# Cardinal-Cryptography/zk-apps

Hardware: AMD Instinct MI355X
Metric: shielder_withdraw_groth16_proofs_per_sec_2^20_constraints (higher is better)
Workload: dtype int: signed 28-bit limbs in 32-bit words, 64-bit column accumulators (Fr 255-bit / Fq 381-bit Montgomery); 1 GPU; single withdraw-shaped Groth16 proof, N=2^20 (7 Fr NTTs, 4 G1 MSM + 1 G2 MSM of 2^20-1 terms), 1 proof per step per GPU; relation=update_note (withdraw) with Poseidon-5 hashing, chain-padded to N, curve=BLS12-381, independent_proofs_per_rank=171, distinct_witnesses_per_rank=64, fresh_r_s_per_proof=True, proofs_in_flight_per_gpu=3, msm_schedule=A | B1 (over r*z) + L + H reduced together | B2 (G2)

## Files before the change

include/zkmi_testing.h:

```cpp
#ifndef ZKMI_TESTING_H
#define ZKMI_TESTING_H
#include "zkmi.h"
#ifdef __cplusplus
extern "C" {
#endif

int32_t zkmi_bases_g1_synthetic(zkmi_ctx* ctx, uint64_t n, zkmi_bases_g1** out);
int32_t zkmi_bases_g2_synthetic(zkmi_ctx* ctx, uint64_t n, zkmi_bases_g2** out);
int32_t zkmi_bases_g1_synthetic_range(zkmi_ctx* ctx, uint64_t first, uint64_t n, zkmi_bases_g1** out);
int32_t zkmi_bn254_bases_synthetic(zkmi_ctx* ctx, uint64_t n, zkmi_bn_bases** out);

int32_t zkmi_shielder_r1cs(uint32_t log_n, zkmi_r1cs** out);
int32_t zkmi_shielder_witness(uint32_t log_n, uint64_t seed, uint8_t* out_z );
int32_t zkmi_shielder_witness_from_input(uint32_t log_n, const zkmi_update_note_input* in, uint8_t* out_z);

int32_t zkmi_selftest_fq28(uint64_t seed, uint32_t iters, uint32_t* out_mismatches);
int32_t zkmi_selftest_assembly(uint64_t seed, uint32_t iters, uint32_t* out_mismatches);
int32_t zkmi_selftest_host_pool(uint32_t callers, uint32_t jobs, uint32_t* out_mismatches);
int32_t zkmi_selftest_poseidon(int32_t field, uint64_t seed, uint32_t iters, uint32_t* out_mismatches);
int32_t zkmi_selftest_miller_formulas(const uint8_t g1_affine[96], const uint8_t g2_affine[192], uint8_t out_fq12[576]);
int32_t zkmi_selftest_final_exp_formulas(const uint8_t in_fq12[576], uint8_t out_chain[576], uint8_t out_plain[576]);
int32_t zkmi_verify_each_kernel_ms(float out_ms[3]);
int32_t zkmi_verify_batch_phases(double out_ms[7]);
int32_t zkmi_selftest_quad_add(zkmi_ctx* ctx, uint64_t seed, uint32_t n, uint32_t* out_mismatches);
int32_t zkmi_selftest_msm_g1_sum2_dev(zkmi_ctx* ctx, const void* d_scalars_a, const void* d_scalars_b, uint64_t n,
                                      const zkmi_bases_g1* bases, uint8_t out_affine[96]);

#ifdef __cplusplus
}
#endif
#endif
```

zk-apps_amd/csrc/field28.hpp:

```cpp
#pragma once
#include "field.hpp"

namespace zkmi {

struct Fq28Params {
  static constexpr int NL = 14;
  static constexpr int N32 = 12;
  static constexpr uint32_t INV = 0xffcfffdu;
  static constexpr int32_t MOD[14] = {0xfffaaab, 0xfefffff, 0x3ffffb9, 0xfffeb15, 0x6241eab, 0xa0f6b0f, 0xf6730d2,
                                      0xf38512b, 0x4774b84, 0x4bacd76, 0xba7b643, 0xe69a4b1, 0x1ea397f, 0x001a011};
  static constexpr int32_t ONE[14] = {0x347fcb8, 0xd800000, 0x002b119, 0x0cde6d2, 0xc7212e0, 0x83a2090, 0x037669f,
                                      0xda0f73e, 0x9b09b42, 0x1297bb0, 0x515d98f, 0x012ca7c, 0x659fcfa, 0x000577a};
  static constexpr int32_t R2[14] = {0x10370ed, 0x6d1c345, 0xe243d62, 0xec45c53, 0x3b1d65a, 0x093317d, 0xb4f36a0,
                                     0x5d74088, 0xc10ea72, 0x865d118, 0x7320a75, 0xfd5cd50, 0xcc8a759, 0x000c8d4};
};

struct Fr28Params {
  static constexpr int NL = 10;
  static constexpr int N32 = 8;
  static constexpr uint32_t INV = 0xfffffffu;
  static constexpr int32_t MOD[10] = {0x0000001, 0xffffff0, 0xe5bfeff, 0xa402fff, 0x80553bd,
                                      0x0809a1d, 0x83339d8, 0x299d7d4, 0x3eda753, 0x0000007};
  static constexpr int32_t ONE[10] = {0xdcaaf6c, 0x355093f, 0x8209402, 0x41e37a6, 0x135587d,
                                      0x26172ba, 0x6854f56, 0x3973f39, 0xbc66e55, 0x0000006};
// ... 496 lines not shown
  __device__ __forceinline__ static void mul_cols(int64_t* T, const Fq2P& a, const Fq2P& b, bool negate) {
    constexpr int NL = Fq28::NL;
    const bool o = odd();
    {
      const Fq28 pb = partner(b.v);
      Fq28 X = sel(o, pb, b.v);
      if (negate) X = negl(X);
#pragma unroll
      for (int i = 0; i < NL; i++)
#pragma unroll
        for (int j = 0; j < NL; j++) T[i + j] += (int64_t)a.v.l[i] * X.l[j];
    }
    {
      const Fq28 pa = partner(a.v);
      Fq28 Y = sel(o, b.v, negl(partner(b.v)));
      if (negate) Y = negl(Y);
#pragma unroll
      for (int i = 0; i < NL; i++)
#pragma unroll
        for (int j = 0; j < NL; j++) T[i + j] += (int64_t)pa.l[i] * Y.l[j];
    }
  }
  __device__ __forceinline__ static void operands(const Fq2P& a, const Fq2P& b, bool negate, Fq28& X, Fq28& pa, Fq28& Y) {
    const bool o = odd();
    const Fq28 pb = partner(b.v);
    X = sel(o, pb, b.v);
    Y = sel(o, b.v, negl(pb));
    if (negate) {
      X = negl(X);
      Y = negl(Y);
    }
    pa = partner(a.v);
  }
  __device__ __forceinline__ friend Fq2P operator*(const Fq2P& a, const Fq2P& b) {
#if defined(ZK_FIPS28)
    {
      Fq28 X, pa, Y;
      operands(a, b, false, X, pa, Y);
      return {Fq28::fips<true>(a.v, X, pa, Y)};
    }
#endif
    int64_t T[2 * Fq28::NL];
#pragma unroll
    for (int i = 0; i < 2 * Fq28::NL; i++) T[i] = 0;
    mul_cols(T, a, b, false);
    return {Fq28::reduce(T)};
  }
  __device__ __forceinline__ Fq2P sqr() const {
    const bool o = odd();
    const Fq28 p = partner(v);
    const Fq28 X = sel(o, p.add_lazy(p), v.add_lazy(p));
    const Fq28 Y = sel(o, v, v.sub_lazy(p));
    return {Fq28::mul_inline(X, Y)};
  }
};
__device__ __forceinline__ Fq2P f_mul_sub_mul(const Fq2P& a, const Fq2P& b, const Fq2P& c, const Fq2P& d) {
#if defined(ZK_FIPS28)
  {
    Fq28 X1, pa, Y1, X2, pc, Y2;
    Fq2P::operands(a, b, false, X1, pa, Y1);
    Fq2P::operands(c, d, true, X2, pc, Y2);
    const Fq28* A[4] = {&a.v, &pa, &c.v, &pc};
    const Fq28* B[4] = {&X1, &Y1, &X2, &Y2};
    return {Fq28::fipsn<4>(A, B)};
  }
#endif
  int64_t T[2 * Fq28::NL];
#pragma unroll
  for (int i = 0; i < 2 * Fq28::NL; i++) T[i] = 0;
  Fq2P::mul_cols(T, a, b, false);
  Fq2P::mul_cols(T, c, d, true);
  return {Fq28::reduce(T)};
}
__device__ __forceinline__ Fq2P f_signed_sub_lazy(const Fq2P& a, uint32_t m, const Fq2P& b) {
  Fq28 r;
#pragma unroll
  for (int i = 0; i < Fq28::NL; i++) r.l[i] = (int32_t)(((uint32_t)a.v.l[i] ^ m) - m) - b.v.l[i];
  r.carry();
  return {r};
}
__device__ __forceinline__ Fq2P f_x3(const Fq2P& rr, const Fq2P& ppp, const Fq2P& q) {
  return {f_x3(rr.v, ppp.v, q.v)};
}
#endif

ZK_HD Fq28 fq28_from_fq(const Fq& a) {
  Fq c = a.from_mont();
  return Fq28::from_canonical(c.l);
}
ZK_HD Fq fq_from_fq28(const Fq28& a) {
  Fq c;
  a.to_canonical(c.l);
  return c.to_mont();
}
ZK_HD BnFq28 fq28_from_fq(const BnFq& a) {
  BnFq c = a.from_mont();
  return BnFq28::from_canonical(c.l);
}
ZK_HD BnFq fq_from_fq28(const BnFq28& a) {
  BnFq c;
  a.to_canonical(c.l);
  return c.to_mont();
}
ZK_HD BnFr28 fr28_from_fr(const BnFr& a) {
  BnFr c = a.from_mont();
  return BnFr28::from_canonical(c.l);
}
ZK_HD Fq2_28 fq28_from_fq(const Fq2& a) { return {fq28_from_fq(a.c0), fq28_from_fq(a.c1)}; }
ZK_HD Fq2 fq_from_fq28(const Fq2_28& a) { return {fq_from_fq28(a.c0), fq_from_fq28(a.c1)}; }

}
```

zk-apps_amd/csrc/msm_impl.hpp:

```cpp
#pragma once
#include <stdlib.h>
#include <functional>
#include <type_traits>
#include <vector>
#include "curve.hpp"
#include "host_pool.hpp"
#include "msm.hpp"

namespace zkmi {

static inline uint64_t msm_max_segments(uint64_t buckets) { return (buckets / 16 > (1u << 16) ? buckets / 16 : (1u << 16)) + 1; }
constexpr int MSM_SEG2_LOG = 4;
constexpr uint32_t MSM_SEG2_MIN_SEGS = 256;
constexpr int MSM_TREE_T = 128;
constexpr uint32_t MSM_STAGE_PTS = 16384;
constexpr uint32_t MSM_STAGE_PTS_1 = 4096;
constexpr uint32_t MSM_HEAVY = 256;

template <class T>
__device__ __forceinline__ T load_vec(const T* p) {
  static_assert(sizeof(T) % 16 == 0, "16-byte multiple");
  T r;
  const uint4* s = reinterpret_cast<const uint4*>(p);
  uint4* d = reinterpret_cast<uint4*>(&r);
#pragma unroll
  for (unsigned i = 0; i < sizeof(T) / 16; i++) d[i] = s[i];
  return r;
}
template <class T>
__device__ __forceinline__ void store_vec(T* p, const T& v) {
  static_assert(sizeof(T) % 16 == 0, "16-byte multiple");
  const uint4* s = reinterpret_cast<const uint4*>(&v);
  uint4* d = reinterpret_cast<uint4*>(p);
#pragma unroll
  for (unsigned i = 0; i < sizeof(T) / 16; i++) d[i] = s[i];
}

typedef __attribute__((address_space(3))) void* lds_ptr_t;
typedef const __attribute__((address_space(1))) void* glb_ptr_t;


__device__ __forceinline__ Fq28 ld_comp(const Fq28* p) {
  Fq28 r;
  const uint2* q = reinterpret_cast<const uint2*>(p);
#pragma unroll
  for (int i = 0; i < 7; i++) {
    const uint2 w = q[i];
    r.l[2 * i] = (int32_t)w.x;
    r.l[2 * i + 1] = (int32_t)w.y;
  }
  return r;
}
__device__ __forceinline__ void st_comp(Fq28* p, const Fq28& v) {
  uint2* q = reinterpret_cast<uint2*>(p);
#pragma unroll
  for (int i = 0; i < 7; i++) q[i] = make_uint2((uint32_t)v.l[2 * i], (uint32_t)v.l[2 * i + 1]);
}


template <class F>
__device__ __forceinline__ bool madd_generic(XYZZ<F>& acc, const Affine<F>& p, uint32_t negmask = 0) {
  F pp_ = f_sub_lazy(p.x * acc.zz, acc.x);
  F r = f_signed_sub_lazy(p.y * acc.zzz, negmask, acc.y);
  F pp = pp_.sqr();
  F rr = r.sqr();
  if (pp.is_zero()) return false;
  F ppp = pp_ * pp;
  acc.zz = acc.zz * pp;
  acc.zzz = acc.zzz * ppp;
  F q = acc.x * pp;
  acc.x = f_x3(rr, ppp, q);
  acc.y = f_mul_sub_mul(r, f_sub_lazy(q, acc.x), acc.y, ppp);
  return true;
}
template <class F>
__device__ __forceinline__ bool madd_affine_pair(XYZZ<F>& acc, const Affine<F>& p, uint32_t negmask = 0) {
  F pp_ = f_sub_lazy(p.x, acc.x);
  F r = f_signed_sub_lazy(p.y, negmask, acc.y);
  F pp = pp_.sqr();
  F rr = r.sqr();
  if (pp.is_zero()) return false;
  F ppp = pp_ * pp;
  F q = acc.x * pp;
  acc.x = f_x3(rr, ppp, q);
  acc.y = f_mul_sub_mul(r, f_sub_lazy(q, acc.x), acc.y, ppp);
  acc.zz = pp;
  acc.zzz = ppp;
  return true;
}
template <class P>
__device__ __forceinline__ bool affine_is_zero_words(const Affine<Fp28<P>>& p) {
  if (p.y.l[0] != 0) return false;
  uint32_t o = 0;
#pragma unroll
  for (int i = 0; i < P::NL; i++) o |= (uint32_t)p.x.l[i] | (uint32_t)p.y.l[i];
  return o == 0;
}

constexpr int MSM_MULTI_MAX = 4;
struct SortView {
  const uint32_t *begin, *count, *perm, *sorted;
  uint32_t heavy_thr;
};
template <class F, bool MULTI>
struct AccumArgs;
template <class F>
struct AccumArgs<F, false> {
  const Affine<F>* bases_;
  XYZZ<F>* buckets_;
  uint32_t* redo_;
  SortView sort_;
  __device__ __forceinline__ const Affine<F>* bases() const { return bases_; }
  __device__ __forceinline__ XYZZ<F>* buckets() const { return buckets_; }
  __device__ __forceinline__ uint32_t* redo() const { return redo_; }
  __device__ __forceinline__ const SortView& sort() const { return sort_; }
};
template <class F>
struct AccumArgs<F, true> {
  const Affine<F>* bases_[MSM_MULTI_MAX];
  XYZZ<F>* buckets_[MSM_MULTI_MAX];
  uint32_t* redo_[MSM_MULTI_MAX];
  SortView sort_[MSM_MULTI_MAX];
  __device__ __forceinline__ const Affine<F>* bases() const { return bases_[blockIdx.y]; }
  __device__ __forceinline__ XYZZ<F>* buckets() const { return buckets_[blockIdx.y]; }
  __device__ __forceinline__ uint32_t* redo() const { return redo_[blockIdx.y]; }
  __device__ __forceinline__ const SortView& sort() const { return sort_[blockIdx.y]; }
};
template <class F, int W, int BW, bool MULTI = false, bool INTO = false>
__global__ void __launch_bounds__(64 * BW, W)
k_accum_g1_nc(const AccumArgs<F, MULTI> args, uint32_t total_buckets) {
  const Affine<F>* __restrict__ const bases = args.bases();
  XYZZ<F>* __restrict__ const buckets = args.buckets();
  uint32_t* __restrict__ const redo = args.redo();
  const uint32_t* __restrict__ const begin = args.sort().begin;
  const uint32_t* __restrict__ const count = args.sort().count;
  const uint32_t* __restrict__ const perm = args.sort().perm;
  const uint32_t* __restrict__ const sorted = args.sort().sorted;
  const uint32_t heavy_thr = args.sort().heavy_thr;
  constexpr int CHUNKS = sizeof(Affine<F>) / 16;
  __shared__ uint4 tile[BW][CHUNKS][64];
  const uint32_t t = blockIdx.x * blockDim.x + threadIdx.x;
  const uint32_t wave = threadIdx.x >> 6, lane = threadIdx.x & 63;
  if (t >= total_buckets) return;
  const uint32_t b = perm[t];
  const uint32_t cnt = count[b];
  if (cnt > heavy_thr) return;
  const uint32_t beg = begin[b], end = beg + cnt;
  auto fetch = [&](uint32_t v) {
    const char* src = reinterpret_cast<const char*>(bases + (v & 0x7fffffffu));
#pragma unroll
    for (int q = 0; q < CHUNKS; q++)
      __builtin_amdgcn_global_load_lds((glb_ptr_t)(src + 16 * q), (lds_ptr_t)&tile[wave][q][0], 16, 0, 0);
  };
  auto take = [&](Affine<F>& p) {
    uint4* d = reinterpret_cast<uint4*>(&p);
#pragma unroll
    for (int q = 0; q < CHUNKS; q++) d[q] = tile[wave][q][lane];
    asm volatile("s_waitcnt lgkmcnt(0)" ::: "memory");
  };
  XYZZ<F> acc;
  uint32_t j = beg;
  for (;; j++) {
    if (j >= end) {
      if constexpr (!INTO) store_vec(buckets + b, XYZZ<F>::infinity());
      return;
    }
    const uint32_t v = sorted[j];
    Affine<F> p = load_vec(bases + (v & 0x7fffffffu));
// ... 101 lines not shown
  const uint32_t* __restrict__ const sorted = args.sort().sorted;
  const uint32_t heavy_thr = args.sort().heavy_thr;
  constexpr int CHUNKS = sizeof(Affine<F>) / 16;
  __shared__ uint4 tile[BW][CHUNKS][64];
  const uint32_t gt = blockIdx.x * blockDim.x + threadIdx.x;
  const uint32_t t = gt >> 1, sub = gt & 1u;
  const uint32_t wave = threadIdx.x >> 6, lane = threadIdx.x & 63;
  if (t >= total_buckets) return;
  const uint32_t b = perm[t];
  const uint32_t cnt = count[b];
  if (cnt > heavy_thr) return;
  const uint32_t beg = begin[b], end = beg + cnt;
  auto fetch = [&](uint32_t v) {
    const char* src = reinterpret_cast<const char*>(bases + (v & 0x7fffffffu));
#pragma unroll
    for (int q = 0; q < CHUNKS; q++)
      __builtin_amdgcn_global_load_lds((glb_ptr_t)(src + 16 * q), (lds_ptr_t)&tile[wave][q][0], 16, 0, 0);
  };
  auto take = [&](Affine<F>& p) {
    uint4* d = reinterpret_cast<uint4*>(&p);
#pragma unroll
    for (int q = 0; q < CHUNKS; q++) d[q] = tile[wave][q][lane];
    asm volatile("s_waitcnt lgkmcnt(0)" ::: "memory");
  };
  XYZZ<F> acc = XYZZ<F>::infinity();
  bool has = false, bad = false;
  uint32_t j = beg + sub;
  for (; j < end; j += 2) {
    const uint32_t v = sorted[j];
    Affine<F> p = load_vec(bases + (v & 0x7fffffffu));
    if (affine_is_zero_words(p)) continue;
    if (v >> 31) p.y = p.y.neg();
    acc.x = p.x;
    acc.y = p.y;
    acc.zz = F::one();
    acc.zzz = F::one();
    has = true;
    j += 2;
    break;
  }
  uint32_t v_cur = 0, v_next = 0;
  if (j < end) {
    v_cur = sorted[j];
    fetch(v_cur);
    if (j + 2 < end) v_next = sorted[j + 2];
  }
  for (; j < end; j += 2) {
    Affine<F> p;
    take(p);
    const uint32_t v = v_cur;
    if (j + 2 < end) {
      fetch(v_next);
      v_cur = v_next;
      if (j + 4 < end) v_next = sorted[j + 4];
    }
    if (affine_is_zero_words(p)) continue;
    if (!madd_generic(acc, p, 0u - (v >> 31))) {
      bad = true;
      break;
    }
  }
  const uint32_t flags = (has ? 1u : 0u) | (bad ? 2u : 0u);
  const uint32_t pflags = (uint32_t)__shfl_xor((int)flags, 1);
  XYZZ<F> o;
#pragma unroll
  for (int i = 0; i < F::NL; i++) {
    o.x.l[i] = __shfl_xor(acc.x.l[i], 1);
    o.y.l[i] = __shfl_xor(acc.y.l[i], 1);
    o.zz.l[i] = __shfl_xor(acc.zz.l[i], 1);
    o.zzz.l[i] = __shfl_xor(acc.zzz.l[i], 1);
  }
  if (sub != 0) return;
  bool redo_it = ((flags | pflags) & 2u) != 0;
  if (!redo_it) {
    if (has && (pflags & 1u)) redo_it = !add_generic(acc, o);
    else if (!has) acc = (pflags & 1u) ? o : XYZZ<F>::infinity();
  }
  if (redo_it)
    redo[1 + atomicAdd(redo, 1u)] = b;
  else
    store_vec(buckets + b, acc);
}

template <int W, int BW>
__global__ void __launch_bounds__(64 * BW, W)
k_accum_g2_nc(const Affine<Fq2_28>* __restrict__ bases, const uint32_t* __restrict__ begin,
              const uint32_t* __restrict__ count, const uint32_t* __restrict__ perm,
              const uint32_t* __restrict__ sorted, XYZZ<Fq2_28>* __restrict__ buckets, uint32_t total_buckets,
              uint32_t heavy_thr, uint32_t* __restrict__ redo) {
  const uint32_t gt = blockIdx.x * blockDim.x + threadIdx.x;
  const uint32_t t = gt >> 1, comp = gt & 1u;
  if (t >= total_buckets) return;
  const uint32_t b = perm[t];
  const uint32_t cnt = count[b];
  if (cnt > heavy_thr) return;
  const uint32_t beg = begin[b], end = beg + cnt;
  Fq28* dst = reinterpret_cast<Fq28*>(buckets + b);
  auto load_point = [&](uint32_t v, Affine<Fq2P>& p) {
    const Fq28* src = reinterpret_cast<const Fq28*>(bases + (v & 0x7fffffffu));
    p.x.v = ld_comp(src + comp);
    p.y.v = ld_comp(src + 2 + comp);
    uint32_t o = (uint32_t)p.y.v.l[0];
    o |= (uint32_t)__builtin_amdgcn_mov_dpp((int)o, 0xB1, 0xF, 0xF, true);
    if (o != 0) return false;
#pragma unroll
    for (int i = 0; i < Fq28::NL; i++) o |= (uint32_t)p.x.v.l[i] | (uint32_t)p.y.v.l[i];
    o |= (uint32_t)__builtin_amdgcn_mov_dpp((int)o, 0xB1, 0xF, 0xF, true);
    return o == 0;
  };
  XYZZ<Fq2P> acc;
  uint32_t j = beg;
  for (;; j++) {
    if (j >= end) {
      const Fq28 z = Fq28::zero();
      for (int k = 0; k < 4; k++) st_comp(dst + 2 * k + comp, z);
      return;
    }
    Affine<Fq2P> p;
    const uint32_t v = sorted[j];
    if (load_point(v, p)) continue;
    acc.x = p.x;
    acc.y = (v >> 31) ? p.y.neg() : p.y;
    j++;
    break;
  }
  bool paired = false;
  for (; j < end && !paired; j++) {
    Affine<Fq2P> p;
    const uint32_t v = sorted[j];
    if (load_point(v, p)) continue;
    if (!madd_affine_pair(acc, p, 0u - (v >> 31))) {
      if (comp == 0) redo[1 + atomicAdd(redo, 1u)] = b;
      return;
    }
    paired = true;
  }
  if (!paired) {
    acc.zz = Fq2P::one();
    acc.zzz = Fq2P::one();
  }
  for (; j < end; j++) {
    Affine<Fq2P> p;
    const uint32_t v = sorted[j];
    if (load_point(v, p)) continue;
    if (!madd_generic(acc, p, 0u - (v >> 31))) {
      if (comp == 0) redo[1 + atomicAdd(redo, 1u)] = b;
      return;
    }
  }
  st_comp(dst + comp, acc.x.v);
  st_comp(dst + 2 + comp, acc.y.v);
  st_comp(dst + 4 + comp, acc.zz.v);
  st_comp(dst + 6 + comp, acc.zzz.v);
}

template <int UNUSED = 0>
__global__ void __launch_bounds__(64, 1)
k_accum_g2_split2(const Affine<Fq2_28>* __restrict__ bases, const uint32_t* __restrict__ begin, const uint32_t* __restrict__ count,
                  const uint32_t* __restrict__ perm, const uint32_t* __restrict__ sorted, XYZZ<Fq2_28>* __restrict__ buckets,
                  uint32_t total_buckets, uint32_t heavy_thr, uint32_t* __restrict__ redo) {
  const uint32_t gt = blockIdx.x * blockDim.x + threadIdx.x;
  const uint32_t t = gt >> 2, sub = (gt >> 1) & 1u, comp = gt & 1u;
  if (t >= total_buckets) return;
  const uint32_t b = perm[t];
  const uint32_t cnt = count[b];
  if (cnt > heavy_thr) return;
  const uint32_t beg = begin[b], end = beg + cnt;
  Fq28* dst = reinterpret_cast<Fq28*>(buckets + b);
  auto load_point = [&](uint32_t v, Affine<Fq2P>& p) {
    const Fq28* src = reinterpret_cast<const Fq28*>(bases + (v & 0x7fffffffu));
    p.x.v = ld_comp(src + comp);
    p.y.v = ld_comp(src + 2 + comp);
    uint32_t o = (uint32_t)p.y.v.l[0];
    o |= (uint32_t)__builtin_amdgcn_mov_dpp((int)o, 0xB1, 0xF, 0xF, true);
    if (o != 0) return false;
#pragma unroll
    for (int i = 0; i < Fq28::NL; i++) o |= (uint32_t)p.x.v.l[i] | (uint32_t)p.y.v.l[i];
    o |= (uint32_t)__builtin_amdgcn_mov_dpp((int)o, 0xB1, 0xF, 0xF, true);
    return o == 0;
  };
  XYZZ<Fq2P> acc = XYZZ<Fq2P>::infinity();
  bool has = false, bad = false;
  uint32_t j = beg + sub;
  for (; j < end; j += 2) {
    Affine<Fq2P> p;
    const uint32_t v = sorted[j];
    if (load_point(v, p)) continue;
    acc.x = p.x;
    acc.y = (v >> 31) ? p.y.neg() : p.y;
    acc.zz = Fq2P::one();
    acc.zzz = Fq2P::one();
    has = true;
    j += 2;
    break;
  }
  for (; j < end; j += 2) {
    Affine<Fq2P> p;
    const uint32_t v = sorted[j];
    if (load_point(v, p)) continue;
    if (!madd_generic(acc, p, 0u - (v >> 31))) {
      bad = true;
      break;
    }
  }
  const uint32_t flags = (has ? 1u : 0u) | (bad ? 2u : 0u);
  const uint32_t pflags = (uint32_t)__shfl_xor((int)flags, 2);
  XYZZ<Fq2P> o;
#pragma unroll
  for (int i = 0; i < Fq28::NL; i++) {
    o.x.v.l[i] = __shfl_xor(acc.x.v.l[i], 2);
    o.y.v.l[i] = __shfl_xor(acc.y.v.l[i], 2);
    o.zz.v.l[i] = __shfl_xor(acc.zz.v.l[i], 2);
    o.zzz.v.l[i] = __shfl_xor(acc.zzz.v.l[i], 2);
  }
  if (sub != 0) return;
  bool redo_it = ((flags | pflags) & 2u) != 0;
  if (!redo_it) {
    if (has && (pflags & 1u)) redo_it = !add_generic(acc, o);
    else if (!has) acc = (pflags & 1u) ? o : XYZZ<Fq2P>::infinity();
  }
  if (redo_it) {
    if (comp == 0) redo[1 + atomicAdd(redo, 1u)] = b;
  } else {
    st_comp(dst + comp, acc.x.v);
    st_comp(dst + 2 + comp, acc.y.v);
    st_comp(dst + 4 + comp, acc.zz.v);
    st_comp(dst + 6 + comp, acc.zzz.v);
  }
}

template <class F>
// ... 229 lines not shown
    for (int q = 0; q < CHUNKS; q++) __builtin_amdgcn_global_load_lds((glb_ptr_t)(src + 16 * q), (lds_ptr_t)&tile[q][0], 16, 0, 0);
  };
  auto take = [&](Affine<F>& p) {
    uint4* d = reinterpret_cast<uint4*>(&p);
#pragma unroll
    for (int q = 0; q < CHUNKS; q++) d[q] = tile[q][lane];
    asm volatile("s_waitcnt lgkmcnt(0)" ::: "memory");
  };
  for (uint32_t it = blockIdx.x; it < n_items; it += gridDim.x) {
    const uint32_t e = heavy_plan_entry(ent, n_ent, it);
    const uint32_t beg = ent[4 * e + 1], cnt = ent[4 * e + 2], first = ent[4 * e + 3];
    const uint32_t w0 = beg + (it - first) * 64u * pl;
    const uint32_t w1 = (w0 + 64u * pl < beg + cnt) ? w0 + 64u * pl : beg + cnt;
    XYZZ<F>* const dst = pool + (size_t)it * 64 + lane;
    XYZZ<F> acc;
    uint32_t j = w0 + lane;
    bool have = false;
    for (; j < w1; j += 64) {
      const uint32_t v = sorted[j];
      Affine<F> p = load_vec(bases + (v & 0x7fffffffu));
      if (affine_is_zero_words(p)) continue;
      if (v >> 31) p.y = p.y.neg();
      acc.x = p.x;
      acc.y = p.y;
      have = true;
      j += 64;
      break;
    }
    if (!have) {
      store_vec(dst, XYZZ<F>::infinity());
      continue;
    }
    uint32_t v_cur = 0, v_next = 0;
    if (j < w1) {
      v_cur = sorted[j];
      fetch(v_cur);
      if (j + 64 < w1) v_next = sorted[j + 64];
    }
    bool bad = false, paired = false;
    if (j < w1) {
      Affine<F> p;
      take(p);
      const uint32_t v = v_cur;
      if (j + 64 < w1) {
        fetch(v_next);
        v_cur = v_next;
        if (j + 128 < w1) v_next = sorted[j + 128];
      }
      j += 64;
      if (!affine_is_zero_words(p)) {
        bad = !madd_affine_pair(acc, p, 0u - (v >> 31));
        paired = true;
      }
    }
    if (!paired) {
      acc.zz = F::one();
      acc.zzz = F::one();
    }
    if (bad) j = w1;
    for (; j < w1; j += 64) {
      Affine<F> p;
      take(p);
      const uint32_t v = v_cur;
      if (j + 64 < w1) {
        fetch(v_next);
        v_cur = v_next;
        if (j + 128 < w1) v_next = sorted[j + 128];
      }
      if (affine_is_zero_words(p)) continue;
      if (!madd_generic(acc, p, 0u - (v >> 31))) {
        bad = true;
        break;
      }
    }
    if (bad) store_vec(dst, heavy_marker<F>());
    else store_vec(dst, acc);
  }
}

template <int W>
__global__ void __launch_bounds__(64, W)
k_accum_heavy_nc_g2(const Affine<Fq2_28>* __restrict__ bases, const uint32_t* __restrict__ sorted, const uint32_t* __restrict__ hplan,
                    XYZZ<Fq2_28>* __restrict__ pool) {
  if (hplan[3] != 0) return;
  const uint32_t n_items = hplan[0], pl = hplan[1], n_ent = hplan[2];
  const uint32_t* __restrict__ const ent = hplan + 4;
  const uint32_t pair = threadIdx.x >> 1, comp = threadIdx.x & 1u;
  auto load_point = [&](uint32_t v, Affine<Fq2P>& p) {
    const Fq28* src = reinterpret_cast<const Fq28*>(bases + (v & 0x7fffffffu));
    p.x.v = ld_comp(src + comp);
    p.y.v = ld_comp(src + 2 + comp);
    uint32_t o = (uint32_t)p.y.v.l[0];
    o |= (uint32_t)__builtin_amdgcn_mov_dpp((int)o, 0xB1, 0xF, 0xF, true);
    if (o != 0) return false;
#pragma unroll
    for (int i = 0; i < Fq28::NL; i++) o |= (uint32_t)p.x.v.l[i] | (uint32_t)p.y.v.l[i];
    o |= (uint32_t)__builtin_amdgcn_mov_dpp((int)o, 0xB1, 0xF, 0xF, true);
    return o == 0;
  };
  for (uint32_t it = blockIdx.x; it < n_items; it += gridDim.x) {
    const uint32_t e = heavy_plan_entry(ent, n_ent, it);
    const uint32_t beg = ent[4 * e + 1], cnt = ent[4 * e + 2], first = ent[4 * e + 3];
    const uint32_t w0 = beg + (it - first) * 32u * pl;
    const uint32_t w1 = (w0 + 32u * pl < beg + cnt) ? w0 + 32u * pl : beg + cnt;
    Fq28* const dst = reinterpret_cast<Fq28*>(pool + (size_t)it * 32 + pair);
    XYZZ<Fq2P> acc;
    uint32_t j = w0 + pair;
    bool have = false, bad = false;
    for (; j < w1; j += 32) {
      Affine<Fq2P> p;
      const uint32_t v = sorted[j];
      if (load_point(v, p)) continue;
      acc.x = p.x;
      acc.y = (v >> 31) ? p.y.neg() : p.y;
      have = true;
      j += 32;
      break;
    }
    if (have) {
      bool paired = false;
      for (; j < w1 && !paired && !bad; j += 32) {
        Affine<Fq2P> p;
        const uint32_t v = sorted[j];
        if (load_point(v, p)) continue;
        if (madd_affine_pair(acc, p, 0u - (v >> 31))) paired = true;
        else bad = true;
      }
      if (!paired) {
        acc.zz = Fq2P::one();
        acc.zzz = Fq2P::one();
      }
      for (; j < w1 && !bad; j += 32) {
        Affine<Fq2P> p;
        const uint32_t v = sorted[j];
        if (load_point(v, p)) continue;
        if (!madd_generic(acc, p, 0u - (v >> 31))) bad = true;
      }
    }
    if (!have || bad) {
      const Fq28 z = Fq28::zero();
      Fq28 mk = z;
      mk.l[0] = (bad && comp == 0) ? 1 : 0;
      st_comp(dst + comp, z);
      st_comp(dst + 2 + comp, z);
      st_comp(dst + 4 + comp, z);
      st_comp(dst + 6 + comp, mk);
    } else {
      st_comp(dst + comp, acc.x.v);
      st_comp(dst + 2 + comp, acc.y.v);
      st_comp(dst + 4 + comp, acc.zz.v);
      st_comp(dst + 6 + comp, acc.zzz.v);
    }
  }
}

constexpr uint32_t MSM_HSPLIT_MAX = 1024;
constexpr uint32_t MSM_HPOOL = MSM_HEAVY_CAP * MSM_HSPLIT;
__device__ __forceinline__ uint32_t heavy_nsplit(uint32_t h, uint32_t count, uint32_t pts, uint32_t item0) {
  if (h >= MSM_HEAVY_CAP) return 1u;
  uint32_t n = (count + pts - 1) / pts;
  n = n < 1 ? 1 : (n > MSM_HSPLIT_MAX ? MSM_HSPLIT_MAX : n);
  if (item0 + n > MSM_HPOOL) n = 1;
  return n;
}
template <class L>
__device__ __forceinline__ void accum_heavy_body(const typename L::Base* __restrict__ bases, const uint32_t* __restrict__ begin,
                                                 const uint32_t* __restrict__ count, const uint32_t* __restrict__ heavy,
                                                 const uint32_t* __restrict__ sorted, typename L::Stored* __restrict__ buckets,
                                                 typename L::Stored* __restrict__ heavy_partial, uint32_t* __restrict__ ticket,
                                                 uint32_t into, uint32_t h_first, uint32_t h_limit, const uint32_t* __restrict__ hplan,
                                                 const typename L::Stored* __restrict__ pool_nc) {
  typedef typename L::P P;
  extern __shared__ __align__(16) unsigned char lds_raw[];
  typename L::Stored* sh = reinterpret_cast<typename L::Stored*>(lds_raw);
  __shared__ uint32_t is_last;
  const uint32_t pt = threadIdx.x / L::LANES, comp = threadIdx.x % L::LANES, npt = blockDim.x / L::LANES;
  constexpr uint32_t PER_ITEM = 64 / L::LANES;
  const bool pmode = hplan != nullptr && hplan[3] == 0;
  const uint32_t* __restrict__ const ent = hplan + 4;
  const uint32_t pl_nc = pmode ? hplan[1] : 0u;
  auto partial_at = [&](uint32_t h, uint32_t j) {
    P v = L::load(pool_nc + j, comp);
    bool empty;
    if (L::is_marker(v, comp, &empty)) {
      const uint32_t it = j / PER_ITEM, ln = j % PER_ITEM;
      const uint32_t beg = ent[4 * h + 1], cnt = ent[4 * h + 2], first = ent[4 * h + 3];
      const uint32_t w0 = beg + (it - first) * PER_ITEM * pl_nc;
      const uint32_t w1 = (w0 + PER_ITEM * pl_nc < beg + cnt) ? w0 + PER_ITEM * pl_nc : beg + cnt;
      v = P::infinity();
      for (uint32_t jj = w0 + ln; jj < w1; jj += PER_ITEM) v.madd(L::load_affine(bases, sorted[jj], comp));
    } else if (empty) {
      v = P::infinity();
    }
    return v;
  };
  const uint32_t n_heavy = pmode ? hplan[2] : (heavy[0] < h_limit ? heavy[0] : h_limit);
  const uint32_t n_wg = gridDim.x * gridDim.y, wg = blockIdx.y * gridDim.x + blockIdx.x;
  uint32_t item0 = 0;
  const bool tail = h_first >= MSM_HEAVY_CAP;
  for (uint32_t h = tail ? h_first + wg : h_first; h < n_heavy; h += tail ? n_wg : 1u) {
    const uint32_t b = pmode ? ent[4 * h] : heavy[1 + h];
    const uint32_t cnt = pmode ? (ent[4 * (h + 1) + 3] - ent[4 * h + 3]) * PER_ITEM : count[b];
    const uint32_t beg0 = pmode ? ent[4 * h + 3] * PER_ITEM : begin[b];
    const uint32_t nsplit = tail ? 1u : heavy_nsplit(h, cnt, 4 * MSM_TREE_T / L::LANES, item0);
    const uint32_t base = item0;
    const uint32_t r0 = tail ? 0u : (wg + n_wg - base % n_wg) % n_wg;
    item0 += nsplit;
    for (uint32_t r = r0; r < nsplit; r += n_wg) {
      uint32_t beg = beg0, end = beg0 + cnt;
      if (nsplit > 1) {
        const uint32_t len = (cnt + nsplit - 1) / nsplit;
        const uint32_t sb = beg + r * len;
        end = (sb + len < end) ? sb + len : end;
        beg = sb < end ? sb : end;
      }
      P acc = P::infinity();
      if (pmode) {
        for (uint32_t j = beg + pt; j < end; j += npt) acc.add(partial_at(h, j));
      } else {
// ... 897 lines not shown
```

zk-apps_amd/csrc/selftest.hip:

```cpp
#include "ctx.hpp"
#include "curve.hpp"
#include "field28.hpp"

using namespace zkmi;

namespace {
struct Rng {
  uint64_t s;
  uint64_t next() {
    s += 0x9E3779B97F4A7C15ull;
    uint64_t z = s;
    z = (z ^ (z >> 30)) * 0xBF58476D1CE4E5B9ull;
    z = (z ^ (z >> 27)) * 0x94D049BB133111EBull;
    return z ^ (z >> 31);
  }
  Fq fq() {
    Fq a;
    for (int i = 0; i < 12; i += 2) {
      uint64_t v = next();
      a.l[i] = (uint32_t)v;
      a.l[i + 1] = (uint32_t)(v >> 32);
    }
    a.l[11] &= 0x0fffffffu;
    return a;
// ... 41 lines not shown
      Fq2_28 X = {A, B}, Y = {C, A * B};
      Fq2 m = x * y, q2 = x.sqr(), chain = (m - q2) * x + y.dbl();
      Fq2_28 M = X * Y, Q2 = X.sqr(), CH = (M - Q2) * X + Y.dbl();
      if (fq_from_fq28(M) != m) bad++;
      if (fq_from_fq28(Q2) != q2) bad++;
      if (fq_from_fq28(CH) != chain) bad++;
      if (!(X * Y - Y * X).is_zero()) bad++;
      if ((X * Y).is_zero() != m.is_zero()) bad++;
    }
    {
      Affine<Fq> p1 = {a, b}, p2 = {c, a * c};
      XYZZ<Fq> h = XYZZ<Fq>::from_affine(p1);
      h.madd(p2);
      XYZZ<Fq> h2 = h;
      h2.madd(p1);
      h.add(h2);
      Affine<Fq28> P1 = {A, B}, P2 = {C, A * C};
      XYZZ<Fq28> d = XYZZ<Fq28>::from_affine(P1);
      d.madd(P2);
      XYZZ<Fq28> d2 = d;
      d2.madd(P1);
      d.add(d2);
      if (fq_from_fq28(d.x) != h.x || fq_from_fq28(d.y) != h.y || fq_from_fq28(d.zz) != h.zz ||
          fq_from_fq28(d.zzz) != h.zzz)
        bad++;
      Affine<Fq2> q1 = {{a, b}, {c, a}}, q2 = {{b, c}, {a * b, c}};
      XYZZ<Fq2> g = XYZZ<Fq2>::from_affine(q1);
      g.madd(q2);
      XYZZ<Fq2> g2 = g;
      g2.madd(q1);
      g.add(g2);
      Affine<Fq2_28> Q1 = {{A, B}, {C, A}}, Q2 = {{B, C}, {A * B, C}};
      XYZZ<Fq2_28> e = XYZZ<Fq2_28>::from_affine(Q1);
      e.madd(Q2);
      XYZZ<Fq2_28> e2 = e;
      e2.madd(Q1);
      e.add(e2);
      if (fq_from_fq28(e.x) != g.x || fq_from_fq28(e.y) != g.y || fq_from_fq28(e.zz) != g.zz ||
          fq_from_fq28(e.zzz) != g.zzz)
        bad++;
    }
    if (fq_from_fq28(A.add_lazy(B) * C.sub_lazy(A)) != (a + b) * (c - a)) bad++;
  }
  *out_mismatches = bad;
  return ZKMI_OK;
}
#endif

#include <atomic>
#include <thread>
#include <vector>
#include "host_pool.hpp"
#ifdef ZKMI_TESTING
extern "C" int32_t zkmi_selftest_host_pool(uint32_t callers, uint32_t jobs, uint32_t* out_mismatches) {
  if (!out_mismatches || callers == 0 || callers > 32) return ZKMI_ERR_BAD_ARG;
  std::atomic<uint32_t> bad{0};
  auto caller = [&](uint32_t c) {
    Rng rng{0x9001u + c};
    for (uint32_t j = 0; j < jobs; j++) {
      const uint32_t n = 1 + (uint32_t)(rng.next() % 64), width = 1 + (uint32_t)(rng.next() % 17);
      std::vector<std::atomic<uint32_t>> hits(n);
      for (auto& h : hits) h.store(0);
      std::atomic<uint64_t> sum{0};
      HostPool::instance().run(n, width, [&](uint32_t i) {
        hits[i].fetch_add(1);
        uint64_t v = i + 1;
        for (int k = 0; k < 200; k++) v = v * 6364136223846793005ull + 1442695040888963407ull;
        sum.fetch_add((v & 1) + i + 1);
      });
      uint64_t lo = (uint64_t)n * (n + 1) / 2;
      for (uint32_t i = 0; i < n; i++)
        if (hits[i].load() != 1) bad.fetch_add(1);
      if (sum.load() < lo || sum.load() > lo + n) bad.fetch_add(1);
    }
  };
  std::vector<std::thread> th;
  for (uint32_t c = 1; c < callers; c++) th.emplace_back(caller, c);
  caller(0);
  for (auto& t : th) t.join();
  *out_mismatches = bad.load();
  return ZKMI_OK;
}
#endif
```

Before: 60.03 proofs/s.

## Prefetch G2 bases via LDS tiles and reuse prepared Fq2 operands in madd

G2 bucket accumulation kernels (normal and heavy) now load the next base point asynchronously into an LDS tile with global_load_lds while the current madd runs, replacing per-iteration direct global loads. Fq2 multiplications in the XYZZ madd formulas precompute the DPP-shuffled/negated right operand (Fq2PPrep) and the partner left operand once, so operands reused across several products skip repeated cross-lane shuffles. A paired squaring routine is also added. This costs extra LDS per block and more live registers for the prepared operands, which may reduce occupancy. A selftest is added for the new arithmetic.

Measured after the change: 60.48 proofs/s, median of 6. Within noise of the previous version (+0.8%).

```diff
diff --git a/include/zkmi_testing.h b/include/zkmi_testing.h
--- a/include/zkmi_testing.h
+++ b/include/zkmi_testing.h
@@ -23,6 +23,7 @@
 int32_t zkmi_verify_each_kernel_ms(float out_ms[3]);
 int32_t zkmi_verify_batch_phases(double out_ms[7]);
 int32_t zkmi_selftest_quad_add(zkmi_ctx* ctx, uint64_t seed, uint32_t n, uint32_t* out_mismatches);
+int32_t zkmi_selftest_fq2p_prep(zkmi_ctx* ctx, uint64_t seed, uint32_t n, uint32_t* out_mismatches);
 int32_t zkmi_selftest_msm_g1_sum2_dev(zkmi_ctx* ctx, const void* d_scalars_a, const void* d_scalars_b, uint64_t n,
                                       const zkmi_bases_g1* bases, uint8_t out_affine[96]);
 
diff --git a/zk-apps_amd/csrc/field28.hpp b/zk-apps_amd/csrc/field28.hpp
--- a/zk-apps_amd/csrc/field28.hpp
+++ b/zk-apps_amd/csrc/field28.hpp
@@ -602,6 +602,96 @@
 __device__ __forceinline__ Fq2P f_x3(const Fq2P& rr, const Fq2P& ppp, const Fq2P& q) {
   return {f_x3(rr.v, ppp.v, q.v)};
 }
+struct Fq2PPrep {
+  Fq28 X, Y;
+  __device__ __forceinline__ static Fq2PPrep of(const Fq2P& b) {
+    const uint32_t m = Fq2P::odd() ? 0u : 0xffffffffu;
+    Fq2PPrep r;
+#pragma unroll
+    for (int i = 0; i < Fq28::NL; i++) {
+      r.X.l[i] = __builtin_amdgcn_mov_dpp(b.v.l[i], 0xA0, 0xF, 0xF, true);
+      const uint32_t t = (uint32_t)__builtin_amdgcn_mov_dpp(b.v.l[i], 0xF5, 0xF, 0xF, true);
+      r.Y.l[i] = (int32_t)((t ^ m) - m);
+    }
+    return r;
+  }
+  __device__ __forceinline__ static void mul_cols(int64_t* T, const Fq2P& a, const Fq2PPrep& b, bool negate) {
+    constexpr int NL = Fq28::NL;
+    const Fq28 av = negate ? Fq2P::negl(a.v) : a.v;
+#pragma unroll
+    for (int i = 0; i < NL; i++)
+#pragma unroll
+      for (int j = 0; j < NL; j++) T[i + j] += (int64_t)av.l[i] * b.X.l[j];
+    const Fq28 pa = Fq2P::partner(av);
+#pragma unroll
+    for (int i = 0; i < NL; i++)
+#pragma unroll
+      for (int j = 0; j < NL; j++) T[i + j] += (int64_t)pa.l[i] * b.Y.l[j];
+  }
+  __device__ __forceinline__ static void mul_cols(int64_t* T, const Fq28& av, const Fq28& pa, const Fq2PPrep& b) {
+    constexpr int NL = Fq28::NL;
+#pragma unroll
+    for (int i = 0; i < NL; i++)
+#pragma unroll
+      for (int j = 0; j < NL; j++) T[i + j] += (int64_t)av.l[i] * b.X.l[j];
+#pragma unroll
+    for (int i = 0; i < NL; i++)
+#pragma unroll
+      for (int j = 0; j < NL; j++) T[i + j] += (int64_t)pa.l[i] * b.Y.l[j];
+  }
+  __device__ __forceinline__ friend Fq2P operator*(const Fq2P& a, const Fq2PPrep& b) {
+#if defined(ZK_FIPS28)
+    return {Fq28::fips<true>(a.v, b.X, Fq2P::partner(a.v), b.Y)};
+#endif
+    int64_t T[2 * Fq28::NL];
+#pragma unroll
+    for (int i = 0; i < 2 * Fq28::NL; i++) T[i] = 0;
+    mul_cols(T, a, b, false);
+    return {Fq28::reduce(T)};
+  }
+};
+struct Fq2PLeft {
+  Fq28 v, p;
+  __device__ __forceinline__ static Fq2PLeft of(const Fq2P& a) { return {a.v, Fq2P::partner(a.v)}; }
+  __device__ __forceinline__ friend Fq2P operator*(const Fq2PLeft& a, const Fq2PPrep& b) {
+#if defined(ZK_FIPS28)
+    return {Fq28::fips<true>(a.v, b.X, a.p, b.Y)};
+#endif
+    int64_t T[2 * Fq28::NL];
+#pragma unroll
+    for (int i = 0; i < 2 * Fq28::NL; i++) T[i] = 0;
+    Fq2PPrep::mul_cols(T, a.v, a.p, b);
+    return {Fq28::reduce(T)};
+  }
+};
+__device__ __forceinline__ Fq2P f_sqr_pair(const Fq2P& a) {
+  const uint32_t me = Fq2P::odd() ? 0u : 0xffffffffu;
+  Fq28 X, Y;
+#pragma unroll
+  for (int i = 0; i < Fq28::NL; i++) {
+    const int32_t a0 = __builtin_amdgcn_mov_dpp(a.v.l[i], 0xA0, 0xF, 0xF, true);
+    const int32_t p = __builtin_amdgcn_mov_dpp(a.v.l[i], 0xB1, 0xF, 0xF, true);
+    X.l[i] = a0 + p;
+    Y.l[i] = a.v.l[i] - (int32_t)((uint32_t)p & me);
+  }
+  return {Fq28::mul_inline(X, Y)};
+}
+__device__ __forceinline__ Fq2P f_mul_sub_mul(const Fq2P& a, const Fq2PPrep& b, const Fq2P& c, const Fq2PPrep& d) {
+#if defined(ZK_FIPS28)
+  {
+    const Fq28 pa = Fq2P::partner(a.v), nc = Fq2P::negl(c.v), pnc = Fq2P::partner(nc);
+    const Fq28* A[4] = {&a.v, &pa, &nc, &pnc};
+    const Fq28* B[4] = {&b.X, &b.Y, &d.X, &d.Y};
+    return {Fq28::fipsn<4>(A, B)};
+  }
+#endif
+  int64_t T[2 * Fq28::NL];
+#pragma unroll
+  for (int i = 0; i < 2 * Fq28::NL; i++) T[i] = 0;
+  Fq2PPrep::mul_cols(T, a, b, false);
+  Fq2PPrep::mul_cols(T, c, d, true);
+  return {Fq28::reduce(T)};
+}
 #endif
 
 ZK_HD Fq28 fq28_from_fq(const Fq& a) {
diff --git a/zk-apps_amd/csrc/msm_impl.hpp b/zk-apps_amd/csrc/msm_impl.hpp
--- a/zk-apps_amd/csrc/msm_impl.hpp
+++ b/zk-apps_amd/csrc/msm_impl.hpp
@@ -84,6 +84,48 @@
   F q = acc.x * pp;
   acc.x = f_x3(rr, ppp, q);
   acc.y = f_mul_sub_mul(r, f_sub_lazy(q, acc.x), acc.y, ppp);
+  acc.zz = pp;
+  acc.zzz = ppp;
+  return true;
+}
+__device__ __forceinline__ bool madd_generic_from(XYZZ<Fq2P>& acc, const Fq2PLeft& zz, const Fq2PLeft& zzz, const Fq2P& u2, const Fq2P& s2,
+                                                  uint32_t negmask) {
+  const Fq2P pp_ = f_sub_lazy(u2, acc.x);
+  const Fq2P r = f_signed_sub_lazy(s2, negmask, acc.y);
+  const Fq2P pp = f_sqr_pair(pp_);
+  const Fq2P rr = f_sqr_pair(r);
+  if (pp.is_zero()) return false;
+  Fq2P ppp, q;
+  {
+    const Fq2PPrep PP = Fq2PPrep::of(pp);
+    ppp = pp_ * PP;
+    acc.zz = zz * PP;
+    q = acc.x * PP;
+  }
+  const Fq2PPrep PPP = Fq2PPrep::of(ppp);
+  acc.zzz = zzz * PPP;
+  acc.x = f_x3(rr, ppp, q);
+  acc.y = f_mul_sub_mul(r, Fq2PPrep::of(f_sub_lazy(q, acc.x)), acc.y, PPP);
+  return true;
+}
+__device__ __forceinline__ bool madd_generic(XYZZ<Fq2P>& acc, const Affine<Fq2P>& p, uint32_t negmask = 0) {
+  const Fq2PLeft zz = Fq2PLeft::of(acc.zz), zzz = Fq2PLeft::of(acc.zzz);
+  return madd_generic_from(acc, zz, zzz, zz * Fq2PPrep::of(p.x), zzz * Fq2PPrep::of(p.y), negmask);
+}
+__device__ __forceinline__ bool madd_affine_pair(XYZZ<Fq2P>& acc, const Affine<Fq2P>& p, uint32_t negmask = 0) {
+  const Fq2P pp_ = f_sub_lazy(p.x, acc.x);
+  const Fq2P r = f_signed_sub_lazy(p.y, negmask, acc.y);
+  const Fq2P pp = f_sqr_pair(pp_);
+  const Fq2P rr = f_sqr_pair(r);
+  if (pp.is_zero()) return false;
+  Fq2P ppp, q;
+  {
+    const Fq2PPrep PP = Fq2PPrep::of(pp);
+    ppp = pp_ * PP;
+    q = acc.x * PP;
+  }
+  acc.x = f_x3(rr, ppp, q);
+  acc.y = f_mul_sub_mul(r, Fq2PPrep::of(f_sub_lazy(q, acc.x)), acc.y, Fq2PPrep::of(ppp));
   acc.zz = pp;
   acc.zzz = ppp;
   return true;
@@ -351,32 +393,75 @@
     store_vec(buckets + b, acc);
 }
 
+constexpr int G2_TILE_CHUNKS = 8;
+__device__ __forceinline__ void g2_tile_fetch(const Affine<Fq2_28>* bases, uint32_t v, uint32_t comp, uint4 (*tile)[64]) {
+  static_assert(sizeof(Affine<Fq2_28>) == 224 && sizeof(Fq28) == 56, "chunking of g2_tile_fetch / g2_tile_take");
+  const char* src = reinterpret_cast<const char*>(bases + (v & 0x7fffffffu)) + 48 * comp;
+#pragma unroll
+  for (int q = 0; q < 4; q++) {
+    __builtin_amdgcn_global_load_lds((glb_ptr_t)(src + 16 * q), (lds_ptr_t)&tile[q][0], 16, 0, 0);
+    __builtin_amdgcn_global_load_lds((glb_ptr_t)(src + 112 + 16 * q), (lds_ptr_t)&tile[4 + q][0], 16, 0, 0);
+  }
+}
+struct G2Entry {
+  Fq2PPrep x, y;
+  __device__ __forceinline__ Affine<Fq2P> own() const {
+    const bool o = Fq2P::odd();
+    return {{Fq2P::sel(o, x.Y, x.X)}, {Fq2P::sel(o, y.Y, y.X)}};
+  }
+};
+__device__ __forceinline__ bool madd_generic(XYZZ<Fq2P>& acc, const G2Entry& p, uint32_t negmask = 0) {
+  const Fq2PLeft zz = Fq2PLeft::of(acc.zz), zzz = Fq2PLeft::of(acc.zzz);
+  return madd_generic_from(acc, zz, zzz, zz * p.x, zzz * p.y, negmask);
+}
+__device__ __forceinline__ bool g2_tile_take(G2Entry& p, uint32_t lane, uint4 (*tile)[64]) {
+  const char* ce = reinterpret_cast<const char*>(&tile[0][lane & ~1u]);
+  const char* co = reinterpret_cast<const char*>(&tile[0][lane | 1u]);
+  Fq28 x1, y1;
+#pragma unroll
+  for (int i = 0; i < 7; i++) {
+    const char* s0 = ce + 1024 * (i / 2) + 8 * (i & 1);
+    const char* s1 = co + ((i & 1) ? 1024 * ((i + 1) / 2) : 8 + 1024 * (i / 2));
+    const uint2 wx0 = *reinterpret_cast<const uint2*>(s0), wy0 = *reinterpret_cast<const uint2*>(s0 + 4096);
+    const uint2 wx1 = *reinterpret_cast<const uint2*>(s1), wy1 = *reinterpret_cast<const uint2*>(s1 + 4096);
+    p.x.X.l[2 * i] = (int32_t)wx0.x;
+    p.x.X.l[2 * i + 1] = (int32_t)wx0.y;
+    p.y.X.l[2 * i] = (int32_t)wy0.x;
+    p.y.X.l[2 * i + 1] = (int32_t)wy0.y;
+    x1.l[2 * i] = (int32_t)wx1.x;
+    x1.l[2 * i + 1] = (int32_t)wx1.y;
+    y1.l[2 * i] = (int32_t)wy1.x;
+    y1.l[2 * i + 1] = (int32_t)wy1.y;
+  }
+  asm volatile("s_waitcnt lgkmcnt(0)" ::: "memory");
+  const uint32_t m = Fq2P::odd() ? 0u : 0xffffffffu;
+#pragma unroll
+  for (int i = 0; i < Fq28::NL; i++) {
+    p.x.Y.l[i] = (int32_t)(((uint32_t)x1.l[i] ^ m) - m);
+    p.y.Y.l[i] = (int32_t)(((uint32_t)y1.l[i] ^ m) - m);
+  }
+  uint32_t o = (uint32_t)p.y.X.l[0] | (uint32_t)y1.l[0];
+  if (o != 0) return false;
+#pragma unroll
+  for (int i = 0; i < Fq28::NL; i++) o |= (uint32_t)p.x.X.l[i] | (uint32_t)x1.l[i] | (uint32_t)p.y.X.l[i] | (uint32_t)y1.l[i];
+  return o == 0;
+}
 template <int W, int BW>
 __global__ void __launch_bounds__(64 * BW, W)
 k_accum_g2_nc(const Affine<Fq2_28>* __restrict__ bases, const uint32_t* __restrict__ begin,
               const uint32_t* __restrict__ count, const uint32_t* __restrict__ perm,
               const uint32_t* __restrict__ sorted, XYZZ<Fq2_28>* __restrict__ buckets, uint32_t total_buckets,
               uint32_t heavy_thr, uint32_t* __restrict__ redo) {
+  __shared__ uint4 tile[BW][G2_TILE_CHUNKS][64];
   const uint32_t gt = blockIdx.x * blockDim.x + threadIdx.x;
   const uint32_t t = gt >> 1, comp = gt & 1u;
+  const uint32_t wave = threadIdx.x >> 6, lane = threadIdx.x & 63;
   if (t >= total_buckets) return;
   const uint32_t b = perm[t];
   const uint32_t cnt = count[b];
   if (cnt > heavy_thr) return;
   const uint32_t beg = begin[b], end = beg + cnt;
   Fq28* dst = reinterpret_cast<Fq28*>(buckets + b);
-  auto load_point = [&](uint32_t v, Affine<Fq2P>& p) {
-    const Fq28* src = reinterpret_cast<const Fq28*>(bases + (v & 0x7fffffffu));
-    p.x.v = ld_comp(src + comp);
-    p.y.v = ld_comp(src + 2 + comp);
-    uint32_t o = (uint32_t)p.y.v.l[0];
-    o |= (uint32_t)__builtin_amdgcn_mov_dpp((int)o, 0xB1, 0xF, 0xF, true);
-    if (o != 0) return false;
-#pragma unroll
-    for (int i = 0; i < Fq28::NL; i++) o |= (uint32_t)p.x.v.l[i] | (uint32_t)p.y.v.l[i];
-    o |= (uint32_t)__builtin_amdgcn_mov_dpp((int)o, 0xB1, 0xF, 0xF, true);
-    return o == 0;
-  };
   XYZZ<Fq2P> acc;
   uint32_t j = beg;
   for (;; j++) {
@@ -385,37 +470,68 @@
       for (int k = 0; k < 4; k++) st_comp(dst + 2 * k + comp, z);
       return;
     }
+    const uint32_t v = sorted[j];
+    const Fq28* src = reinterpret_cast<const Fq28*>(bases + (v & 0x7fffffffu));
     Affine<Fq2P> p;
-    const uint32_t v = sorted[j];
-    if (load_point(v, p)) continue;
+    p.x.v = ld_comp(src + comp);
+    p.y.v = ld_comp(src + 2 + comp);
+    uint32_t o = 0;
+#pragma unroll
+    for (int i = 0; i < Fq28::NL; i++) o |= (uint32_t)p.x.v.l[i] | (uint32_t)p.y.v.l[i];
+    o |= (uint32_t)__builtin_amdgcn_mov_dpp((int)o, 0xB1, 0xF, 0xF, true);
+    if (o == 0) continue;
     acc.x = p.x;
     acc.y = (v >> 31) ? p.y.neg() : p.y;
     j++;
     break;
   }
+  bool bad = false;
+  uint32_t v_cur = 0, v_next = 0;
+  if (j < end) {
+    v_cur = sorted[j];
+    g2_tile_fetch(bases, v_cur, comp, tile[wave]);
+    if (j + 1 < end) v_next = sorted[j + 1];
+  }
   bool paired = false;
-  for (; j < end && !paired; j++) {
-    Affine<Fq2P> p;
-    const uint32_t v = sorted[j];
-    if (load_point(v, p)) continue;
-    if (!madd_affine_pair(acc, p, 0u - (v >> 31))) {
-      if (comp == 0) redo[1 + atomicAdd(redo, 1u)] = b;
-      return;
-    }
-    paired = true;
+  if (j < end) {
+    G2Entry p;
+    const bool inf = g2_tile_take(p, lane, tile[wave]);
+    const uint32_t v = v_cur;
+    if (j + 1 < end) {
+      g2_tile_fetch(bases, v_next, comp, tile[wave]);
+      v_cur = v_next;
+      if (j + 2 < end) v_next = sorted[j + 2];
+    }
+    j++;
+    if (!inf) {
+      bad = !madd_affine_pair(acc, p.own(), 0u - (v >> 31));
+      paired = true;
+    }
   }
   if (!paired) {
     acc.zz = Fq2P::one();
     acc.zzz = Fq2P::one();
   }
-  for (; j < end; j++) {
-    Affine<Fq2P> p;
-    const uint32_t v = sorted[j];
-    if (load_point(v, p)) continue;
+  if (bad) j = end;
+  const uint32_t* sp = sorted + j;
+  for (uint32_t rem = end - j; rem > 0; rem--, sp++) {
+    G2Entry p;
+    const bool inf = g2_tile_take(p, lane, tile[wave]);
+    const uint32_t v = v_cur;
+    if (rem > 1) {
+      g2_tile_fetch(bases, v_next, comp, tile[wave]);
+      v_cur = v_next;
+      if (rem > 2) v_next = sp[2];
+    }
+    if (inf) continue;
     if (!madd_generic(acc, p, 0u - (v >> 31))) {
-      if (comp == 0) redo[1 + atomicAdd(redo, 1u)] = b;
-      return;
-    }
+      bad = true;
+      break;
+    }
+  }
+  if (bad) {
+    if (comp == 0) redo[1 + atomicAdd(redo, 1u)] = b;
+    return;
   }
   st_comp(dst + comp, acc.x.v);
   st_comp(dst + 2 + comp, acc.y.v);
@@ -811,22 +927,11 @@
 __global__ void __launch_bounds__(64, W)
 k_accum_heavy_nc_g2(const Affine<Fq2_28>* __restrict__ bases, const uint32_t* __restrict__ sorted, const uint32_t* __restrict__ hplan,
                     XYZZ<Fq2_28>* __restrict__ pool) {
+  __shared__ uint4 tile[G2_TILE_CHUNKS][64];
   if (hplan[3] != 0) return;
   const uint32_t n_items = hplan[0], pl = hplan[1], n_ent = hplan[2];
   const uint32_t* __restrict__ const ent = hplan + 4;
-  const uint32_t pair = threadIdx.x >> 1, comp = threadIdx.x & 1u;
-  auto load_point = [&](uint32_t v, Affine<Fq2P>& p) {
-    const Fq28* src = reinterpret_cast<const Fq28*>(bases + (v & 0x7fffffffu));
-    p.x.v = ld_comp(src + comp);
-    p.y.v = ld_comp(src + 2 + comp);
-    uint32_t o = (uint32_t)p.y.v.l[0];
-    o |= (uint32_t)__builtin_amdgcn_mov_dpp((int)o, 0xB1, 0xF, 0xF, true);
-    if (o != 0) return false;
-#pragma unroll
-    for (int i = 0; i < Fq28::NL; i++) o |= (uint32_t)p.x.v.l[i] | (uint32_t)p.y.v.l[i];
-    o |= (uint32_t)__builtin_amdgcn_mov_dpp((int)o, 0xB1, 0xF, 0xF, true);
-    return o == 0;
-  };
+  const uint32_t lane = threadIdx.x, pair = threadIdx.x >> 1, comp = threadIdx.x & 1u;
   for (uint32_t it = blockIdx.x; it < n_items; it += gridDim.x) {
     const uint32_t e = heavy_plan_entry(ent, n_ent, it);
     const uint32_t beg = ent[4 * e + 1], cnt = ent[4 * e + 2], first = ent[4 * e + 3];
@@ -837,9 +942,16 @@
     uint32_t j = w0 + pair;
     bool have = false, bad = false;
     for (; j < w1; j += 32) {
+      const uint32_t v = sorted[j];
+      const Fq28* src = reinterpret_cast<const Fq28*>(bases + (v & 0x7fffffffu));
       Affine<Fq2P> p;
-      const uint32_t v = sorted[j];
-      if (load_point(v, p)) continue;
+      p.x.v = ld_comp(src + comp);
+      p.y.v = ld_comp(src + 2 + comp);
+      uint32_t o = 0;
+#pragma unroll
+      for (int i = 0; i < Fq28::NL; i++) o |= (uint32_t)p.x.v.l[i] | (uint32_t)p.y.v.l[i];
+      o |= (uint32_t)__builtin_amdgcn_mov_dpp((int)o, 0xB1, 0xF, 0xF, true);
+      if (o == 0) continue;
       acc.x = p.x;
       acc.y = (v >> 31) ? p.y.neg() : p.y;
       have = true;
@@ -847,23 +959,47 @@
       break;
     }
     if (have) {
+      uint32_t v_cur = 0, v_next = 0;
+      if (j < w1) {
+        v_cur = sorted[j];
+        g2_tile_fetch(bases, v_cur, comp, tile);
+        if (j + 32 < w1) v_next = sorted[j + 32];
+      }
       bool paired = false;
-      for (; j < w1 && !paired && !bad; j += 32) {
-        Affine<Fq2P> p;
-        const uint32_t v = sorted[j];
-        if (load_point(v, p)) continue;
-        if (madd_affine_pair(acc, p, 0u - (v >> 31))) paired = true;
-        else bad = true;
+      if (j < w1) {
+        G2Entry p;
+        const bool inf = g2_tile_take(p, lane, tile);
+        const uint32_t v = v_cur;
+        if (j + 32 < w1) {
+          g2_tile_fetch(bases, v_next, comp, tile);
+          v_cur = v_next;
+          if (j + 64 < w1) v_next = sorted[j + 64];
+        }
+        j += 32;
+        if (!inf) {
+          bad = !madd_affine_pair(acc, p.own(), 0u - (v >> 31));
+          paired = true;
+        }
       }
       if (!paired) {
         acc.zz = Fq2P::one();
         acc.zzz = Fq2P::one();
       }
-      for (; j < w1 && !bad; j += 32) {
-        Affine<Fq2P> p;
-        const uint32_t v = sorted[j];
-        if (load_point(v, p)) continue;
-        if (!madd_generic(acc, p, 0u - (v >> 31))) bad = true;
+      if (bad) j = w1;
+      for (; j < w1; j += 32) {
+        G2Entry p;
+        const bool inf = g2_tile_take(p, lane, tile);
+        const uint32_t v = v_cur;
+        if (j + 32 < w1) {
+          g2_tile_fetch(bases, v_next, comp, tile);
+          v_cur = v_next;
+          if (j + 64 < w1) v_next = sorted[j + 64];
+        }
+        if (inf) continue;
+        if (!madd_generic(acc, p, 0u - (v >> 31))) {
+          bad = true;
+          break;
+        }
       }
     }
     if (!have || bad) {
diff --git a/zk-apps_amd/csrc/selftest.hip b/zk-apps_amd/csrc/selftest.hip
--- a/zk-apps_amd/csrc/selftest.hip
+++ b/zk-apps_amd/csrc/selftest.hip
@@ -147,3 +147,93 @@
   return ZKMI_OK;
 }
 #endif
+
+#ifdef ZKMI_TESTING
+namespace {
+constexpr int FQ2P_IN = 4, FQ2P_OUT = 8;
+__global__ void __launch_bounds__(64) k_fq2p_prep(const Fq2_28* __restrict__ in, Fq2_28* __restrict__ out, uint32_t n) {
+  const uint32_t gt = blockIdx.x * blockDim.x + threadIdx.x, i = gt >> 1, comp = gt & 1u;
+  if (i >= n) return;
+  const Fq28* s = reinterpret_cast<const Fq28*>(in + (size_t)FQ2P_IN * i);
+  const Fq2P a = {s[comp]}, b = {s[2 + comp]}, c = {s[4 + comp]}, d = {s[6 + comp]};
+  Fq28* o = reinterpret_cast<Fq28*>(out + (size_t)FQ2P_OUT * i);
+  const Fq2PPrep B = Fq2PPrep::of(b), D = Fq2PPrep::of(d);
+  o[0 + comp] = (a * b).v;
+  o[2 + comp] = (a * B).v;
+  o[4 + comp] = (Fq2PLeft::of(a) * B).v;
+  o[6 + comp] = f_mul_sub_mul(a, b, c, d).v;
+  o[8 + comp] = f_mul_sub_mul(a, B, c, D).v;
+  o[10 + comp] = a.sqr().v;
+  o[12 + comp] = f_sqr_pair(a).v;
+  o[14 + comp] = f_sqr_pair(f_sub_lazy(a, c)).v;
+}
+bool same_limbs(const Fq2_28& x, const Fq2_28& y) {
+  for (int i = 0; i < Fq28::NL; i++)
+    if (x.c0.l[i] != y.c0.l[i] || x.c1.l[i] != y.c1.l[i]) return false;
+  return true;
+}
+}
+
+extern "C" int32_t zkmi_selftest_fq2p_prep(zkmi_ctx* ctx, uint64_t seed, uint32_t n, uint32_t* out_mismatches) {
+  if (!ctx || !out_mismatches || n == 0 || n > (1u << 20)) return ZKMI_ERR_BAD_ARG;
+  if (hipSetDevice(ctx->device) != hipSuccess) return ZKMI_ERR_HIP;
+  Rng rng{seed};
+  std::vector<Fq2> h((size_t)FQ2P_IN * n);
+  std::vector<Fq2_28> in((size_t)FQ2P_IN * n), out((size_t)FQ2P_OUT * n);
+  const Fq2 zero = {Fq::zero(), Fq::zero()}, one = {Fq::one(), Fq::zero()}, u = {Fq::zero(), Fq::one()};
+  for (uint32_t i = 0; i < n; i++) {
+    Fq2 a = {rng.fq(), rng.fq()}, b = {rng.fq(), rng.fq()}, c = {rng.fq(), rng.fq()}, d = {rng.fq(), rng.fq()};
+    switch (i % 16) {
+      case 1: b = zero; break;
+      case 2: a = zero; break;
+      case 3: b = one; break;
+      case 4: b = u; break;
+      case 5: b = a; break;
+      case 6: c = a, d = b; break;
+      case 7: c = b, d = a; break;
+      case 8: b = zero - a; break;
+      case 9: d = zero; break;
+      case 10: a.c1 = Fq::zero(), b.c1 = Fq::zero(); break;
+      case 11: a.c0 = Fq::zero(), b.c0 = Fq::zero(); break;
+      case 12: c = a; break;
+      case 13: d = one, c = one; break;
+      default: break;
+    }
+    const Fq2 v[FQ2P_IN] = {a, b, c, d};
+    for (int k = 0; k < FQ2P_IN; k++) {
+      h[(size_t)FQ2P_IN * i + k] = v[k];
+      in[(size_t)FQ2P_IN * i + k] = fq28_from_fq(v[k]);
+    }
+  }
+  Fq2_28 *gin = nullptr, *gout = nullptr;
+  int32_t rc = ZKMI_OK;
+  uint32_t bad = 0;
+  if (hipMalloc(&gin, sizeof(Fq2_28) * in.size()) != hipSuccess || hipMalloc(&gout, sizeof(Fq2_28) * out.size()) != hipSuccess ||
+      hipMemcpy(gin, in.data(), sizeof(Fq2_28) * in.size(), hipMemcpyHostToDevice) != hipSuccess) {
+    rc = ZKMI_ERR_HIP;
+  } else {
+    hipLaunchKernelGGL(k_fq2p_prep, dim3((2 * n + 63) / 64), dim3(64), 0, ctx->stream, gin, gout, n);
+    if (hipStreamSynchronize(ctx->stream) != hipSuccess ||
+        hipMemcpy(out.data(), gout, sizeof(Fq2_28) * out.size(), hipMemcpyDeviceToHost) != hipSuccess)
+      rc = ZKMI_ERR_HIP;
+  }
+  if (rc == ZKMI_OK) {
+    for (uint32_t i = 0; i < n; i++) {
+      const Fq2 &a = h[(size_t)FQ2P_IN * i], &b = h[(size_t)FQ2P_IN * i + 1], &c = h[(size_t)FQ2P_IN * i + 2], &d = h[(size_t)FQ2P_IN * i + 3];
+      const Fq2_28* o = &out[(size_t)FQ2P_OUT * i];
+      if (!same_limbs(o[1], o[0])) bad++;
+      if (!same_limbs(o[2], o[0])) bad++;
+      if (!same_limbs(o[4], o[3])) bad++;
+      if (!same_limbs(o[6], o[5])) bad++;
+      if (fq_from_fq28(o[1]) != a * b) bad++;
+      if (fq_from_fq28(o[4]) != a * b - c * d) bad++;
+      if (fq_from_fq28(o[6]) != a.sqr()) bad++;
+      if (fq_from_fq28(o[7]) != (a - c).sqr()) bad++;
+    }
+  }
+  (void)hipFree(gin);
+  (void)hipFree(gout);
+  *out_mismatches = bad;
+  return rc;
+}
+#endif
```
